# klindsay28/Newton-Krylov_OOC

Measured on AMD Instinct MI355X. Metric: GMRES JVPs/sec, py_driver_2d iage (value = value_frozen: products on frozen years, the default; value_reference_semantic: the reference's product, two free-running years, same solver, same run), higher is better.
Workload: dtype f64

## Files before the change

### newton-krylov_ooc_amd/csrc/nk2d_api.hip

```cpp
#include "nk2d_common.h"
#include "nk2d_build_id.h"

#include <algorithm>
#include <cmath>
#include <cstring>
#include <new>

namespace {

template <typename T>
int dev_alloc(nk2d_ctx* c, T** p, size_t n) {
    NK2D_CHECK(c, hipMalloc((void**)p, sizeof(T) * std::max<size_t>(n, 1)));
    NK2D_CHECK(c, hipMemsetAsync(*p, 0, sizeof(T) * std::max<size_t>(n, 1), nk2d_s(c)));
    return 0;
}

int ensure_stage(nk2d_ctx* c, size_t n) {
    if (n <= c->stage_elems) return 0;
    NK2D_CHECK(c, hipStreamSynchronize(nk2d_s(c)));
    if (c->STAGE) NK2D_CHECK(c, hipFree(c->STAGE));
    if (c->hSTAGE) NK2D_CHECK(c, hipHostFree(c->hSTAGE));
    c->STAGE = c->hSTAGE = nullptr;
    c->stage_elems = 0;
    NK2D_CHECK(c, hipMalloc((void**)&c->STAGE, sizeof(double) * n));
// ... 191 lines not shown
    }
    if (key == "pc_panel") {
        if (value != 32.0 && value != 64.0) return nk2d_fail(c, "nk2d_set_option: pc_panel is 32 or 64");
        c->pc_panel = (int)value;
        return 0;
    }
    if (key == "final_fuse") { c->final_fuse = value != 0.0; return 0; }
    if (key == "year_fences") { c->year_fences = value != 0.0; return 0; }
    if (key == "frozen_persistent") { c->frozen_persistent = value != 0.0; return 0; }
    if (key == "frozen_team") { c->frozen_team = value != 0.0; return 0; }
    if (key == "frozen_coef_lds") { c->frozen_coef_lds = (int)value & 63; return 0; }
    if (key == "frozen_sums_poison") { c->frozen_sums_poison = (int)value != 0 ? 1 : 0; return 0; }
    if (key == "frozen_early") { c->frozen_early = (int)value != 0 ? 1 : 0; return 0; }
    if (key == "frozen_stage_exchange") { c->frozen_stage_exchange = (int)value != 0 ? 1 : 0; return 0; }
    if (key == "frozen_xlane") { c->frozen_xlane = (int)value != 0 ? 1 : 0; return 0; }
    if (key == "frozen_by_column") { c->frozen_by_column = (int)value; return 0; }
    if (key == "frozen_cache_after") { c->frozen_cache_after = (int)value; return 0; }
    if (key == "spec_bias") { c->spec_bias = value > 0.0 ? value : 1.0; return 0; }
    if (key == "stream_years") { c->stream_years = (int)value; c->stream_lost = 0; return 0; }
    if (key == "frozen_tape") {
        if (value != 0.0 && value != 1.0) return nk2d_fail(c, "nk2d_set_option: frozen_tape is 0 or 1");
        c->frozen_tape = (int)value;
        return 0;
    }
    if (key == "stream_hist") {
        if (value != 0.0 && value != 1.0) return nk2d_fail(c, "nk2d_set_option: stream_hist is 0 or 1");
        c->stream_hist = (int)value;
        return 0;
    }
    if (key == "stream_hist_mb") {
// ... 406 lines not shown
    c->frozen_forced_years = 0;
    c->frozen_phosphorus = 0;
    c->frozen_phosphorus_shallow = 0;
    c->frozen_phosphorus_shallow_years = 0;
    c->frozen_two_waves_last = 0;
    c->frozen_phosphorus_years = c->frozen_two_waves_years = 0;
    c->frozen_cache_piece_allocs = c->frozen_cache_early_requests = 0;
    c->frozen_coef_lds = 63;
    c->frozen_lds_bits = 0;
    c->frozen_early = NK2D_FROZEN_EARLY_DEFAULT;
    c->frozen_early_bits = 0;
    c->frozen_stage_exchange = NK2D_FROZEN_STAGE_EXCHANGE_DEFAULT;
    c->frozen_stage_exchange_bits = 0;
    c->frozen_xlane = NK2D_FROZEN_XLANE_DEFAULT;
    c->frozen_xlane_bits = 0;
    c->stream_xlane = 0;
    c->stream_xlane_bits = 0;
    c->frozen_by_column = 1;
    c->strm = nullptr;
    c->spec_bias = 1.0;
    c->stream_two_waves = std::getenv("NK2D_STREAM_TWO_WAVES") ? std::atoi(std::getenv("NK2D_STREAM_TWO_WAVES")) : 1;
    c->stream_years = 1;
    c->stream_on = 0;
    c->stream_lost = 0;
    c->stream_cmds = c->stream_launches = c->stream_timeouts = c->stream_years_run = 0;
    c->frozen_tape = 0;
    c->tape = nullptr;
    c->tape_rec = c->tape_foreign = 0;
    c->tape_years_run = c->tape_builds = c->tape_timeouts = c->tape_fallbacks = 0;
    c->frozen_wpb = 2;
// ... 498 lines not shown
        int w = -1, row = -1, lane = -1;
        if (std::sscanf(key.c_str() + 15, "%d_%d_%d", &w, &row, &lane) != 3 || w < 0 || w > 1 || row < 0 || row >= NK2D_XLANE_SELFTEST_ROWS ||
            lane < 0 || lane > 63)
            return nk2d_fail(c, "nk2d_get_counter: unknown counter " + key);
        v = xl_selftest_out[((size_t)w * NK2D_XLANE_SELFTEST_ROWS + row) * 64 + lane];
    }
    else if (key == "frozen_launch_us") v = c->frozen_launch_us;
    else if (key == "frozen_cache_pending") v = nk2d_frozen_cache_pending(c);
    else if (key == "frozen_cache_bytes") v = nk2d_frozen_cache_bytes(c);
    else if (key == "frozen_cache_pieces") v = nk2d_frozen_cache_npieces(c);
    else if (key == "frozen_cache_lean") v = nk2d_frozen_cache_is_lean(c);
    else if (key == "frozen_lds_bits") v = c->frozen_lds_bits;
    else if (key == "frozen_early_bits") v = c->frozen_early_bits;
    else if (key == "frozen_stage_exchange_bits") v = c->frozen_stage_exchange_bits;
    else if (key == "frozen_xlane_bits") v = c->frozen_xlane_bits;
    else if (key == "stream_xlane_bits") v = c->stream_xlane_bits;
    else if (key == "frozen_step_sums_hash") v = c->frozen_step_sums_hash;
    else if (key == "frozen_lean_years") v = c->frozen_lean_years;
    else if (key == "frozen_forced_years") v = c->frozen_forced_years;
    else if (key == "frozen_phosphorus_years") v = c->frozen_phosphorus_years;
    else if (key == "frozen_phosphorus_shallow_years") v = c->frozen_phosphorus_shallow_years;
    else if (key == "frozen_two_waves_years") v = c->frozen_two_waves_years;
    else if (key == "frozen_cache_piece_allocs") v = nk2d_frozen_cache_piece_allocs(c);
    else if (key == "frozen_cache_early_requests") v = c->frozen_cache_early_requests;
    else if (key == "frozen_fallbacks") v = c->frozen_fallbacks;
    else if (key == "frozen_resumes") v = c->frozen_resumes;
    else if (key == "spec_launches_dropped") v = c->cnt_spec_dropped;
    else if (key == "spec_front_launches_dropped") v = c->cnt_front_dropped;
    else if (key == "err_estimates_queued") v = c->cnt_err_queued;
    else if (key == "err_estimates_dropped") v = c->cnt_err_void;
// ... 331 lines not shown
```

### newton-krylov_ooc_amd/csrc/nk2d_bodies.h

```cpp
#pragma once
#include <atomic>
#include <chrono>
#include <cmath>
#include <cstdio>
#include <cstdlib>
#include <cstring>
#include <mutex>
#include <thread>

#include "nk2d_common.h"
#include "nk2d_hostmath.h"


struct DevP {
    int nz, ny, tc, ncol;
    const double *VV, *KH, *WT, *WB, *DZR, *ZM0, *ZM1, *DM, *DMR, *DYR, *BLDMAX;
    double surf[NK2D_MAX_TRACERS], starget[NK2D_MAX_TRACERS], decay[NK2D_MAX_TRACERS], csrc;
    double atol, rtol;
    double ph_hs, ph_mu, ph_sig, ph_rd, ph_rp, ph_vs;
    const double *LIGHT, *UPR;
    const double *SMSREC, *RESTREC;
    int f_sms, f_restore;
    double f_thres_r;
    size_t np;
// ... 1912 lines not shown
                }
                __builtin_amdgcn_s_sleep(1);
            }
            if (lane == 0) *lds_ok = good;
#ifdef NK2D_FROZEN_CLOCKS
            ck_wait += (long long)__builtin_amdgcn_s_memrealtime() - ck_flag;
#endif
        }
        __syncthreads();
#ifdef NK2D_FROZEN_CLOCKS
        ck_match = (long long)__builtin_amdgcn_s_memrealtime();
#endif
        if (fences) __builtin_amdgcn_fence(__ATOMIC_ACQUIRE, "agent");
        return *lds_ok != 0;
    }
    __device__ __forceinline__ bool sync() {
        asm volatile("s_waitcnt vmcnt(0)" ::: "memory");
        if (fences) __builtin_amdgcn_fence(__ATOMIC_RELEASE, "agent");
        __syncthreads();
        ++phase;
        if (threadIdx.x < 64) {
            const int lane = threadIdx.x;
            if (lane == 0) __hip_atomic_store(flags + (size_t)me * 32, phase, __ATOMIC_RELAXED, __HIP_MEMORY_SCOPE_AGENT);
            const int other = (lane == 0) ? left : ((lane == 1) ? right : -1);
            int good = 1;
            long long spins = 0;
            const long long t_begin = (long long)__builtin_amdgcn_s_memrealtime();
            for (;;) {
                unsigned v = phase;
                if (other >= 0) v = __hip_atomic_load(flags + (size_t)other * 32, __ATOMIC_RELAXED, __HIP_MEMORY_SCOPE_AGENT);
// ... 239 lines not shown
    int fences;
    int coef_lds;
#define NK2D_FROZEN_EARLY_OF(coef_lds) (((coef_lds) >> 8) & 1)
#define NK2D_FROZEN_XCHG_OF(coef_lds) (((coef_lds) >> 9) & 1)
#define NK2D_FROZEN_XLANE_OF(coef_lds) (((coef_lds) >> 10) & 1)
    int by_column;
    const double* SRC;
    int upr_on;
};

struct FrozenPieceArgs : FrozenArgs {
    PieceTab T;
};
template <int PIECES> struct FrozenArgOf { typedef FrozenArgs type; };
template <> struct FrozenArgOf<1> { typedef FrozenPieceArgs type; };

template <int E, int KIND, int MP>
__device__ __forceinline__ void tend_at_body(const DevP& P, const double* __restrict__ y, const double* __restrict__ kvp,
                                             double* __restrict__ f, int task, int lane) {
    const int tr = task / P.ny, j = task - tr * P.ny;
    const int cs_col = (j > 0) ? task - 1 : task, cn_col = (j < P.ny - 1) ? task + 1 : task;
    ColCoef<E> cf;
    load_coef<E>(P, j, lane, cf);
    double c[E], cs[E], cn[E], kv[E], ff[E];
    load_col<E, MP>(y, task, lane, c);
    load_col<E, MP>(y, cs_col, lane, cs);
    load_col<E, MP>(y, cn_col, lane, cn);
    load_col<E, MP>(kvp, j, lane, kv);
    tend_col<E, KIND>(P, cf, c, cs, cn, kv, tr, lane, ff);
    if constexpr (KIND == 2) forced_sources<E>(P, kvp, j, lane, c, ff);
// ... 56 lines not shown
```

### newton-krylov_ooc_amd/csrc/nk2d_common.h

```cpp
#pragma once

#include <hip/hip_runtime.h>
#include <stdint.h>
#include <string>
#include <mutex>
#include <vector>

#include "../../include/nk2d.h"

#define NK2D_WAVE 64
#define NK2D_WAVES_PER_BLOCK 4
#define NK2D_BLOCK (NK2D_WAVE * NK2D_WAVES_PER_BLOCK)
#define NK2D_MAX_E 8
#define NK2D_OWN_REC_CAP 65536
#define NK2D_CKPT_EVERY 128


#define NK2D_FROZEN_EARLY_DEFAULT 1
#define NK2D_FROZEN_STAGE_EXCHANGE_DEFAULT 1
#define NK2D_FROZEN_XLANE_DEFAULT 1
#ifndef NK2D_FROZEN_XLANE_MOVES
#define NK2D_FROZEN_XLANE_MOVES 97
#endif
struct nk2d_ctx {
    nk2d_desc d;
    int nz, ny, tc, E, nzp, ncol, nreg;
    int kind;
    size_t nv;
    size_t np;
    int dev;
    hipStream_t stream_;
    std::string err;
    struct nk2d_stream_state* strm;
    int stream_years;
    int stream_two_waves;
// ... 61 lines not shown
    void* frozen_cache;
    int frozen_persistent;
    int frozen_persistent_max_e;
    double frozen_cache_max_gb;
    int64_t frozen_cache_builds, frozen_persistent_years;
    int frozen_team;
    int frozen_wpb;
    int frozen_coef_lds;
    int frozen_lds_bits;
    int frozen_early;
    int frozen_early_bits;
    int frozen_stage_exchange;
    int frozen_stage_exchange_bits;
    int frozen_xlane;
    int frozen_xlane_bits;
    int frozen_by_column;
    int frozen_alloc_async;
    int frozen_cache_after;
    int frozen_cache_pieces;
    double frozen_cache_piece_mb;
    int64_t frozen_cache_piece_rows;
    int frozen_cache_lean;
    int64_t frozen_lean_years;
    uint64_t frozen_lean_mem_key;
    int frozen_forced;
    int64_t frozen_forced_years;
    int frozen_phosphorus;
    int frozen_phosphorus_shallow;
    int64_t frozen_phosphorus_shallow_years;
    int frozen_two_waves_last;
// ... 621 lines not shown
```

### newton-krylov_ooc_amd/csrc/nk2d_frozen.hip

```cpp
#include "nk2d_bodies.h"
#include "nk2d_frozen_plan.h"

#include <algorithm>
#ifdef NK2D_FROZEN_CLOCKS
#include <cstdio>
#endif
#include <vector>

__device__ __forceinline__ RowTabs cache_row_tabs(const CachePiecePtrs& C, int i) {
    const int p = i / C.T.rows;
    return piece_row_tabs(C.C, C.T, C.T.base[p], i - p * C.T.rows);
}

template <int E, int PIECES = 0>
__global__ void __launch_bounds__(NK2D_BLOCK) k_cache_planes(DevP P, const CacheRow* __restrict__ rows, typename CacheArgOf<PIECES>::type C, int n) {
    const int lane = threadIdx.x & 63;
    const long long task = (long long)blockIdx.x * (blockDim.x >> 6) + (threadIdx.x >> 6);
    const long long per_row = 4LL * P.ny;
    if (task >= per_row * n) return;
    const int i = (int)(task / per_row), rem = (int)(task - (long long)i * per_row);
    const int slot = rem / P.ny, j = rem - slot * P.ny;
    const CacheRow& R = rows[i];
    if (slot < 3) {
        double kv[E];
// ... 56 lines not shown
__device__ __forceinline__ void frozen_factor_phase(const DevP& P, const FusedArgs& FA, int wave, int lane, const FinalArgs* fin, const LdsSrc* L,
                                                    int coef_lds, bool w_in_lds, double* piv_lds) {
    if (w_in_lds) newton_fused_body<E, KIND, 1, 1, MPX, FINAL, 3>(P, FA, wave, lane, fin, L);
    else if (coef_lds) newton_fused_body<E, KIND, 1, 1, MPX, FINAL, 1>(P, FA, wave, lane, fin, L);
    else newton_fused_body<E, KIND, 1, 1, MPX, FINAL>(P, FA, wave, lane, fin);
    if (piv_lds) {
        asm volatile("s_waitcnt vmcnt(0)" ::: "memory");
        double v[E];
        load_col<E>(FA.sw.fr_inv, wave, lane, v);
        w_lds_put<E>(piv_lds, 0, lane, v);
    }
}

template <int E, int KIND, int TEAM = 0, int PIECES = 0, int LEAN = 0>
__global__ void __launch_bounds__(NK2D_BLOCK) k_frozen_persistent(DevP P, typename FrozenArgOf<PIECES>::type A) {
#include "nk2d_frozen_body.inc"
}
template <int E, int PIECES>
__global__ void __launch_bounds__(NK2D_BLOCK) __attribute__((amdgpu_waves_per_eu(2, 2))) k_frozen_persistent_w2(DevP P, typename FrozenArgOf<PIECES>::type A) {
    constexpr int KIND = 1, TEAM = 0, LEAN = 1;
#include "nk2d_frozen_body.inc"
}

struct nk2d_frozen_cache {
    uint64_t key = 0;
    int64_t n = 0;
    std::vector<double*> blocks;
    size_t block_rows = 0;
    bool pieces = false, lean = false, src = false;
    double** blocks_dev = nullptr;
    size_t blocks_dev_cap = 0;
    CacheRow* rows_dev = nullptr;
    FrozenRow* frows_dev = nullptr;
    size_t rows_cap = 0;
    std::vector<FrozenRow> frows;
    double* lean_tab = nullptr;
// ... 143 lines not shown
static hipError_t launch_resident(nk2d_ctx* c, K kernel, dim3 grid, dim3 block, DevP& P, ARGS& A, size_t lds_bytes = 0, bool check_only = false) {
    int per_cu = 0;
    hipError_t rc = hipOccupancyMaxActiveBlocksPerMultiprocessor(&per_cu, kernel, (int)block.x, lds_bytes);
    if (rc != hipSuccess) return rc;
    hipDeviceProp_t prop;
    rc = hipGetDeviceProperties(&prop, c->dev);
    if (rc != hipSuccess) return rc;
    if ((long long)per_cu * prop.multiProcessorCount < (long long)grid.x) return hipErrorCooperativeLaunchTooLarge;
    if (check_only) return hipSuccess;
    if (std::getenv("NK2D_DIAG_COOPERATIVE")) {
        void* args[2] = {&P, &A};
        return hipLaunchCooperativeKernel((const void*)kernel, grid, block, args, (unsigned)lds_bytes, nk2d_s(c));
    }
    hipLaunchKernelGGL(kernel, grid, block, lds_bytes, nk2d_s(c), P, A);
    return hipGetLastError();
}

template <int E, int KIND, int TEAM, int PIECES, int LEAN>
static hipError_t launch_frozen_one(nk2d_ctx* c, dim3 grid, DevP& P, typename FrozenArgOf<PIECES>::type& A) {
    const int wpb = TEAM ? NK2D_WAVES_PER_BLOCK : std::max(1, std::min(NK2D_WAVES_PER_BLOCK, c->frozen_wpb));
    const dim3 g = TEAM ? grid : dim3((unsigned)((c->ncol + wpb - 1) / wpb));
    if (!TEAM && E >= 3 && A.by_column)
        return launch_resident(c, k_frozen_persistent<E, KIND, TEAM, PIECES, LEAN>, dim3((unsigned)c->ny), dim3(64 * c->tc), P, A,
                               sizeof(double) * frozen_lds_doubles(E, A.coef_lds, true, c->tc));
    const size_t lds = (!TEAM && E >= 3 && A.coef_lds) ? sizeof(double) * frozen_lds_doubles(E, A.coef_lds, false, wpb) : 0;
    return launch_resident(c, k_frozen_persistent<E, KIND, TEAM, PIECES, LEAN>, g, dim3(64 * wpb), P, A, lds);
}
template <int KIND, int TEAM, int PIECES, int LEAN>
static hipError_t launch_frozen_e(nk2d_ctx* c, dim3 grid, DevP& P, typename FrozenArgOf<PIECES>::type& A) {
    switch (c->E) {
// ... 321 lines not shown
    A.upr_on = (pl.src || pl.phos) ? 1 : 0;
    A.SRC = (pl.src && !pl.pieces) ? fc->blocks[0] + L.oS : nullptr;
    *P = make_devp(c);
    if (pl.src || pl.phos) P->UPR = fc->upr;
    NK2D_TRY(frozen_fit_lds(c, in, pl, &A.coef_lds, &A.by_column));
    c->frozen_lds_bits = A.coef_lds;
    c->frozen_early_bits = (A.coef_lds & 48) == 48 ? c->frozen_early : 0;
    A.coef_lds |= c->frozen_early_bits << 8;
    const bool team_year = c->frozen_team && c->E <= 2 && !pl.phos;
    c->frozen_stage_exchange_bits =
        ((A.coef_lds & 48) == 48 && NK2D_FROZEN_XCHG(c->E, c->kind, team_year, pl.pieces, pl.lean)) ? c->frozen_stage_exchange : 0;
    A.coef_lds |= c->frozen_stage_exchange_bits << 9;
    c->frozen_xlane_bits =
        (c->frozen_stage_exchange_bits != 0 && NK2D_FROZEN_XLANE(c->E, c->kind, team_year, pl.pieces, pl.lean)) ? c->frozen_xlane : 0;
    A.coef_lds |= c->frozen_xlane_bits << 10;
    return 0;
}

static int frozen_launch_year(nk2d_ctx* c, const FrozenPlan& pl, int64_t n, DevP& P, FrozenPieceArgs& A) {
    const bool team = c->frozen_team && c->E <= 2 && !pl.phos;
    const dim3 grid((unsigned)(team ? c->ncol : nk2d_grid(c->ncol)));
    NK2D_CHECK(c, hipMemsetAsync(c->YR_SYNC, 0, yr_sync_bytes(c), nk2d_s(c)));
    NK2D_CHECK(c, hipMemsetAsync(c->YR_OUT, 0, sizeof(double) * 32, nk2d_s(c)));
    NK2D_CHECK(c, hipEventRecord(c->yr_ev[0], nk2d_s(c)));
    {
        struct Turn {
            int waves;
            explicit Turn(int w) : waves(w) { nk2d_turn_take(waves); }
            ~Turn() { nk2d_turn_give(waves); }
        } turn(team ? 4 * c->ncol : c->ncol);
        hipError_t rc = hipErrorInvalidValue;
        bool two = false;
        if (pl.phos) rc = launch_frozen_phos_flavour(c, pl.pieces, P, A, false, &two);
        else if (pl.lean) rc = pl.pieces ? launch_frozen<1, 1>(c, team, grid, P, A) : launch_frozen<0, 1>(c, team, grid, P, static_cast<FrozenArgs&>(A));
        else rc = pl.pieces ? launch_frozen<1, 0>(c, team, grid, P, A) : launch_frozen<0, 0>(c, team, grid, P, static_cast<FrozenArgs&>(A));
        c->frozen_two_waves_last = two ? 1 : 0;
        if (rc == hipErrorCooperativeLaunchTooLarge) { (void)hipGetLastError(); return 1; }
        NK2D_CHECK(c, rc);
        NK2D_CHECK(c, hipEventRecord(c->yr_ev[1], nk2d_s(c)));
        NK2D_CHECK(c, hipMemcpyAsync(c->hYR_OUT, c->YR_OUT, sizeof(double) * 32, hipMemcpyDeviceToHost, nk2d_s(c)));
        NK2D_CHECK(c, hipStreamSynchronize(nk2d_s(c)));
    }
    const double* o = c->hYR_OUT;
    if ((int)o[0] != 0 || (int64_t)o[1] != n) return 2;
#ifdef NK2D_FROZEN_CLOCKS
    std::fprintf(stderr, "frozen clocks (early %d, stage exchange %d, xlane %d): %.0f phases, per phase drain %.3f us, flag store to poll match %.3f us, "
                 "poll match to neighbours loaded %.3f us, rest %.3f us; kernel %.3f ms\n",
                 c->frozen_early_bits, c->frozen_stage_exchange_bits, c->frozen_xlane_bits, o[11], 0.01 * o[8] / o[11], 0.01 * o[9] / o[11], 0.01 * o[12] / o[11],
// ... 75 lines not shown
```

### newton-krylov_ooc_amd/csrc/nk2d_frozen_body.inc

```
    constexpr int XCD = 0, NB = 1;
    __shared__ int lds_ok;
    __shared__ double team_lds[TEAM ? sizeof(TeamLds<E, 3>) / sizeof(double) : 1];
    constexpr int MPX = XCD ? 2 : 1;
    const int lane = threadIdx.x & 63;
    int wg = (int)blockIdx.x;
    const int tw = uni_i((int)(threadIdx.x >> 6));
    const bool by_col = !TEAM && !XCD && NB != 0 && A.by_column != 0;
    const int wave = TEAM ? uni_i(wg) : (by_col ? uni_i(tw * P.ny + wg) : uni_i(wg * (int)(blockDim.x >> 6) + (int)(threadIdx.x >> 6)));
    const bool col_wave = wave < P.ncol && (!by_col || (tw < P.tc && wg < P.ny));
    int nb_left, nb_right;
    if constexpr (TEAM) {
        const int nb_j = wave % P.ny;
        nb_left = (nb_j > 0) ? wg - 1 : -1;
        nb_right = (nb_j < P.ny - 1) ? wg + 1 : -1;
    } else if (by_col) {
        nb_left = (wg > 0) ? wg - 1 : -1;
        nb_right = (wg < P.ny - 1) ? wg + 1 : -1;
    } else {
        const int wpb = (int)(blockDim.x >> 6);
        const int c0 = wg * wpb, cl = min(c0 + wpb - 1, P.ncol - 1);
        nb_left = (c0 % P.ny > 0) ? wg - 1 : -1;
        nb_right = (cl % P.ny < P.ny - 1) ? wg + 1 : -1;
    }
    NeighbourSync nbs{(unsigned*)((char*)A.arrive + 8192), A.abort_flag, wg, nb_left, nb_right, 0u, &lds_ok, A.spin_ticks, A.fences};
// ... 6 lines not shown
    (void)pc_p; (void)pc_r;
#define FZ_Y (swapY ? A.YOLD : A.Y)
#define FZ_YOLD (swapY ? A.Y : A.YOLD)
#define FZ_Z (swapZ ? A.ZN : A.Z)
#define FZ_ZN (swapZ ? A.Z : A.ZN)
#define FZ_SYNC() \
    if (!nbs.sync()) { status = 1; goto finish; }
#define FZ_OWN_DEAD() \
    if constexpr (OWN) { \
        _Pragma("unroll") for (int r_ = 0; r_ < 3; ++r_) { \
            _Pragma("unroll") for (int e_ = 0; e_ < E; ++e_) own.z[r_][e_] = 0.0; \
        } \
    }
    constexpr bool COEF_LDS = NB != 0 && !TEAM && !XCD && E >= 3;
    extern __shared__ double dyn_lds[];
    const bool w_in_lds = COEF_LDS && (A.coef_lds & 2) != 0;
    const bool step_in_lds = COEF_LDS && by_col && (A.coef_lds & 4) != 0;
    const bool piv_in_lds = COEF_LDS && by_col && (A.coef_lds & 8) != 0;
    constexpr bool OWN = COEF_LDS && NK2D_FROZEN_OWN(E, KIND, TEAM, LEAN);
    const int own_bits = OWN && by_col ? (A.coef_lds & 48) : 0;
    (void)own_bits;
    const int nwv = (int)(blockDim.x >> 6);
    double* my_coef;
    double* my_w;
    double* step_lds = nullptr;
    double* my_piv = nullptr;
    double* my_y = nullptr;
    if (by_col) {
        double* p = dyn_lds;
        my_coef = p; p += NK2D_COEF_LDS_DOUBLES(E);
        step_lds = p; p += step_in_lds ? 5 * E * 64 : 0;
        my_w = p + (size_t)tw * (3 * E * 64); p += w_in_lds ? (size_t)nwv * 3 * E * 64 : 0;
        my_piv = p + (size_t)tw * (E * 64); p += piv_in_lds ? (size_t)nwv * E * 64 : 0;
        my_y = p + (size_t)tw * (E * 64);
    } else {
// ... 9 lines not shown
        for (int r = 0; r < 3; ++r) {
#pragma unroll
            for (int e = 0; e < E; ++e) own.z[r][e] = 0.0;
        }
    }
    if constexpr (COEF_LDS) {
        if (A.coef_lds && col_wave && (!by_col || tw == 0)) {
            ColCoef<E> cf;
            load_coef<E>(P, wave % P.ny, lane, cf);
            store_coef_lds<E>(my_coef, lane, cf);
        }
        if (by_col && A.coef_lds) __syncthreads();
    }
    int lds_step = -1;
    (void)lds_step;
    LateNorm late = {0.0, nullptr, (OWN && by_col && own_bits == 48) ? uni_i(NK2D_FROZEN_EARLY_OF(A.coef_lds)) : 0, 0};
    (void)late;
    constexpr bool XCHG = OWN && NK2D_FROZEN_XCHG(E, KIND, TEAM, PIECES, LEAN);
    const int xchg = (XCHG && by_col && own_bits == 48) ? uni_i(NK2D_FROZEN_XCHG_OF(A.coef_lds)) : 0;
    double* const xu0 = XCHG ? (double*)((char*)A.arrive + yr_xchg_offset(P.ncol)) : nullptr;
    (void)xchg; (void)xu0;
    constexpr bool XLANE = XCHG && NK2D_FROZEN_XLANE(E, KIND, TEAM, PIECES, LEAN);
    const int xlane = (XLANE && xchg) ? uni_i(NK2D_FROZEN_XLANE_OF(A.coef_lds)) : 0;
    (void)xlane;
#define FZ_U (swapZ ? xu0 + 3 * nv : xu0)
#define FZ_UN (swapZ ? xu0 : xu0 + 3 * nv)
    if (col_wave && (!TEAM || tw == 0)) {
        double zero[E];
#pragma unroll
        for (int e = 0; e < E; ++e) zero[e] = 0.0;
        if constexpr (XCHG) {
            if (xchg) {
                double y0[E];
                load_col<E, MPX>(FZ_Y, wave, lane, y0);
#pragma unroll
                for (int e = 0; e < E; ++e) y0[e] = y0[e] + zero[e];
#pragma unroll
                for (int i = 0; i < 3; ++i) store_col<E, 1>(FZ_U + i * nv, wave, lane, y0);
            }
// ... 102 lines not shown
                        }
                        }
                        lds_step = i;
                        __syncthreads();
                    }
                }
#ifdef NK2D_FROZEN_CLOCKS
                late.ck_match = nbs.ck_match;
#endif
                if (is_final) {
                    FinalArgs Fin;
                    Fin.ynew = FZ_YOLD;
                    Fin.znext = do_stage ? FZ_ZN : FZ_Z;
                    Fin.x0 = R.x0; Fin.x1 = R.x1; Fin.x2 = R.x2;
                    Fin.nblk_cols = 0;
                    if constexpr (TEAM) {
                        if constexpr (LEAN) {
                            if (col_wave && fac)
                                newton_team_body<E, KIND, 1, 1, 4, 1, MPX>(PK, FA, *reinterpret_cast<TeamLds<E, 3>*>(team_lds), wave, tw, lane, &Fin);
                        }
                        if (col_wave && !fac)
                            newton_team_body<E, KIND, 0, 1, 4, 1, MPX>(P, FA, *reinterpret_cast<TeamLds<E, 3>*>(team_lds), wave, tw, lane, &Fin);
                    } else if (col_wave && fac) {
                        if constexpr (LEAN && COEF_LDS) frozen_factor_phase<E, KIND, MPX, 1>(PK, FA, wave, lane, &Fin, &L, A.coef_lds, w_in_lds, piv_in_lds ? my_piv : nullptr);
                        else if constexpr (LEAN) newton_fused_body<E, KIND, 1, 1, MPX, 1>(PK, FA, wave, lane, &Fin);
                    } else if (col_wave) {
                        bool taken = false;
                        if constexpr (KIND == 0 && E <= 2) {
                            if (m == 1) { newton_single_body<E, MPX, 1>(P, FA, wave, lane, &Fin); taken = true; }
                        }
// ... 9 lines not shown
                            }
                            if (taken) {}
                            else if (own_bits == 48) { newton_fused_body<E, KIND, 0, 1, MPX, 1, 191>(P, FA, wave, lane, &Fin, &L, &own, &late); taken = true; }
                            else if (!PIECES && own_bits == 32) { newton_fused_body<E, KIND, 0, 1, MPX, 1, 47>(P, FA, wave, lane, &Fin, &L, &own); taken = true; }
                            else if (own_bits == 16) { newton_fused_body<E, KIND, 0, 1, MPX, 1, 31>(P, FA, wave, lane, &Fin, &L, &own); FZ_OWN_DEAD() taken = true; }
                        }
                        if constexpr (COEF_LDS) {
                            if (taken) {}
                            else if (step_in_lds && piv_in_lds) { newton_fused_body<E, KIND, 0, 1, MPX, 1, 15>(P, FA, wave, lane, &Fin, &L); FZ_OWN_DEAD() taken = true; }
                            else if (step_in_lds) { newton_fused_body<E, KIND, 0, 1, MPX, 1, 7>(P, FA, wave, lane, &Fin, &L); FZ_OWN_DEAD() taken = true; }
                            else if (w_in_lds) { newton_fused_body<E, KIND, 0, 1, MPX, 1, 3>(P, FA, wave, lane, &Fin, &L); FZ_OWN_DEAD() taken = true; }
                            else if (A.coef_lds) { newton_fused_body<E, KIND, 0, 1, MPX, 1, 1>(P, FA, wave, lane, &Fin, &L); FZ_OWN_DEAD() taken = true; }
                        }
                        if (!taken) { newton_fused_body<E, KIND, 0, 1, MPX, 1>(P, FA, wave, lane, &Fin); FZ_OWN_DEAD() }
                    }
                    swapY ^= 1;
                    if (do_stage) swapZ ^= 1;
                } else {
                    if constexpr (TEAM) {
                        if constexpr (LEAN) {
                            if (col_wave && fac)
                                newton_team_body<E, KIND, 1, 1, 4, 0, MPX>(PK, FA, *reinterpret_cast<TeamLds<E, 3>*>(team_lds), wave, tw, lane, nullptr);
                        }
                        if (col_wave && !fac)
                            newton_team_body<E, KIND, 0, 1, 4, 0, MPX>(P, FA, *reinterpret_cast<TeamLds<E, 3>*>(team_lds), wave, tw, lane, nullptr);
                    } else if (col_wave && fac) {
                        if constexpr (LEAN && COEF_LDS) frozen_factor_phase<E, KIND, MPX, 0>(PK, FA, wave, lane, nullptr, &L, A.coef_lds, w_in_lds, piv_in_lds ? my_piv : nullptr);
                        else if constexpr (LEAN) newton_fused_body<E, KIND, 1, 1, MPX, 0>(PK, FA, wave, lane);
                    } else if (col_wave) {
                        bool taken = false;
                        if constexpr (KIND == 0 && E <= 2) {
                            if (m == 1) { newton_single_body<E, MPX, 0>(P, FA, wave, lane); taken = true; }
                        }
// ... 9 lines not shown
                            }
                            if (taken) {}
                            else if (own_bits == 48) { newton_fused_body<E, KIND, 0, 1, MPX, 0, 191>(P, FA, wave, lane, nullptr, &L, &own, &late); taken = true; }
                            else if (!PIECES && own_bits == 32) { newton_fused_body<E, KIND, 0, 1, MPX, 0, 47>(P, FA, wave, lane, nullptr, &L, &own); taken = true; }
                            else if (own_bits == 16) { newton_fused_body<E, KIND, 0, 1, MPX, 0, 31>(P, FA, wave, lane, nullptr, &L, &own); FZ_OWN_DEAD() taken = true; }
                        }
                        if constexpr (COEF_LDS) {
                            if (taken) {}
                            else if (step_in_lds && piv_in_lds) { newton_fused_body<E, KIND, 0, 1, MPX, 0, 15>(P, FA, wave, lane, nullptr, &L); FZ_OWN_DEAD() taken = true; }
                            else if (step_in_lds) { newton_fused_body<E, KIND, 0, 1, MPX, 0, 7>(P, FA, wave, lane, nullptr, &L); FZ_OWN_DEAD() taken = true; }
                            else if (w_in_lds) { newton_fused_body<E, KIND, 0, 1, MPX, 0, 3>(P, FA, wave, lane, nullptr, &L); FZ_OWN_DEAD() taken = true; }
                            else if (A.coef_lds) { newton_fused_body<E, KIND, 0, 1, MPX, 0, 1>(P, FA, wave, lane, nullptr, &L); FZ_OWN_DEAD() taken = true; }
                        }
                        if (!taken) { newton_fused_body<E, KIND, 0, 1, MPX, 0>(P, FA, wave, lane); FZ_OWN_DEAD() }
                    }
                    if (do_stage && do_update) swapZ ^= 1;
                }
                src = 1 - src;
                if constexpr (OWN) {
                    nbs.publish();
                    if (late.pending) {
                        if (lane == 0) st_mp<MPX>(late.part, late.acc);
                        late.pending = 0;
                    }
                    if (!nbs.wait()) { status = 1; goto finish; }
                } else {
                    FZ_SYNC()
                }
            }
        }
        if (with_err) {
            if (col_wave && (!TEAM || tw == 0)) {
                ErrArgs EA = {};
                EA.sw.JL = J; EA.sw.JU = J + A.C.np; EA.sw.JS = J + 2 * A.C.np; EA.sw.JN = J + 3 * A.C.np; EA.sw.JC = J + 4 * A.C.np;
                EA.sw.fr_inv = LEAN ? A.C.fr_inv : (PIECES ? T.fr_inv : A.C.fr_inv + (size_t)i * nv);
                EA.sw.fr_tab = LEAN ? A.C.fr_tab : (PIECES ? T.fr_tab : A.C.fr_tab + (size_t)i * A.C.ntab);
                EA.sw.xr_old = A.XR[0]; EA.sw.xr_new = A.XR[1];
                EA.f = A.F; EA.z = FZ_Z; EA.y = FZ_Y; EA.nv = nv; EA.h = R.h;
                EA.part = A.STEP_PART + (size_t)(3 * i + 2) * P.ncol;
                EA.stage = 0; EA.last = 1;
// ... 64 lines not shown
```

### newton-krylov_ooc_amd/csrc/nk2d_frozen_plan.h

```cpp
#pragma once

#include <algorithm>
#include <cmath>
#include <cstddef>
#include <cstdint>
#include <initializer_list>

#define NK2D_WAVES_PER_BLOCK 4
#define NK2D_TAB 14
#define NK2D_SCHED_WIDTH 8
#define NK2D_COEF_LDS_DOUBLES(E) ((7 * (E) + 1) * 64)

#define NK2D_FROZEN_OWN(E, KIND, TEAM, LEAN) ((E) >= 5 && (E) <= 7 && ((KIND) == 0 || (KIND) == 2) && !(TEAM) && !(LEAN))
#define NK2D_FROZEN_XCHG(E, KIND, TEAM, PIECES, LEAN) (NK2D_FROZEN_OWN(E, KIND, TEAM, LEAN) && !((E) == 7 && (KIND) == 0 && (PIECES)))
#define NK2D_FROZEN_XLANE(E, KIND, TEAM, PIECES, LEAN) (NK2D_FROZEN_XCHG(E, KIND, TEAM, PIECES, LEAN) && !((E) == 6 && (KIND) == 0 && (PIECES)))

struct FrozenPlanIn {
    int E, kind, tc, ny, ncol;
    size_t np, nv, kv_len;
    int sms_nrec;
    double sink_thres, t0;
    int frozen_persistent, frozen_persistent_max_e, frozen_forced, frozen_phosphorus;
    int frozen_phosphorus_shallow;
    int frozen_cache_lean, frozen_cache_pieces;
    double frozen_cache_piece_mb;
    int64_t frozen_cache_piece_rows;
    double frozen_cache_max_gb;
    int frozen_cache_after, frozen_alloc_async, frozen_err_check;
    int frozen_coef_lds, frozen_by_column, frozen_wpb, frozen_team;
    int factor_fp32, jac_stage_state, hist_n;
// ... 232 lines not shown
```

### newton-krylov_ooc_amd/csrc/nk2d_radau.hip

```cpp
#include "nk2d_common.h"
#include "nk2d_stream.h"

#include <algorithm>
#include <chrono>
#include <cmath>
#include <cstring>
#include <limits>
#include <string>
#include <vector>

namespace {

const double RC[3] = {0.15505102572168222, 0.6449489742783178, 1.0};
const double MU_REAL = 3.637834252744496;
const double MU_CR = 2.6810828736277523, MU_CI = -3.050430199247411;
const int NEWTON_MAXITER = 6;
const double MIN_FACTOR = 0.2, MAX_FACTOR = 10.0;

struct Ctl {
    nk2d_ctx* c;
    double t, t1;
    double h_abs, h_abs_old, err_old;
    bool has_old_h, has_old_err;
    bool current_jac, have_lu, have_dense;
// ... 981 lines not shown
    };
    if (!s.no_persistent && !c->stream_on) {
        std::vector<char> sampled;
        const int prc = nk2d_frozen_persistent(c, sched, n, &sampled);
        if (prc < 0) return prc;
        if (prc == 0) {
            const double* r = sched + (n - 1) * NK2D_SCHED_WIDTH;
            s.t = r[0];
            NK2D_TRY(commit_step(s, r[0], r[1]));
            NK2D_TRY(fetch_sums(0));
            if (first_unconverged(sched, 0) < 0) {
                const int64_t bad_err = first_bad_err(sched, 0, -1, sampled);
                if (bad_err >= 0) return err_failure(bad_err);
                c->frozen_persistent_years++;
                if (nk2d_frozen_cache_is_lean(c)) c->frozen_lean_years++;
                if (c->kind == 2 && (c->E > 4 || (c->d.sms_nrec > 0 && c->d.sink_thres > 0.0))) c->frozen_forced_years++;
                if (c->kind == 1) { c->frozen_phosphorus_years++; c->frozen_two_waves_years += c->frozen_two_waves_last; }
                if (c->kind == 1 && c->E <= 2) c->frozen_phosphorus_shallow_years++;
                return 0;
            }
            return 3;
        }
        if (prc == 2) {
            c->st.nbarrier_timeouts++;
            if (c->kind == 1) c->frozen_fallbacks++;
            return 3;
        }
    }
    int64_t start = 0;
    std::vector<char> err_done((size_t)n, 0);
// ... 215 lines not shown
```

### newton-krylov_ooc_amd/engine.py

```python

import ctypes
import os

import numpy as np

from . import _lib
from .grid import BLDEPTH_MIN, YEAR, bldepth_time_knots


DEFAULT_LIN_TOL = 3.0e-2
DEFAULT_JAC_FRESH = 1
DEFAULT_JAC_STAGE = 1
DEFAULT_GROWTH_CAP = 0.0


def phos_pc_fused_from_env():
    return int(os.environ.get("NK2D_PHOS_PC_FUSED", "0")) != 0


class Nk2dError(RuntimeError):
    pass


class Nk2dFrozenMismatch(Nk2dError):
# ... 163 lines not shown
            self.set_option("frozen_cache_early", float(os.environ["NK2D_FROZEN_CACHE_EARLY"]))
        if "NK2D_FROZEN_CACHE_LEAN" in os.environ:
            self.set_option("frozen_cache_lean", float(os.environ["NK2D_FROZEN_CACHE_LEAN"]))
        if "NK2D_FROZEN_FORCED" in os.environ:
            self.set_option("frozen_forced", float(os.environ["NK2D_FROZEN_FORCED"]))
        if "NK2D_FROZEN_PHOSPHORUS" in os.environ:
            self.set_option("frozen_phosphorus", float(os.environ["NK2D_FROZEN_PHOSPHORUS"]))
        if "NK2D_FROZEN_PHOSPHORUS_SHALLOW" in os.environ:
            self.set_option("frozen_phosphorus_shallow", float(os.environ["NK2D_FROZEN_PHOSPHORUS_SHALLOW"]))
        if "NK2D_FROZEN_EARLY" in os.environ:
            self.set_option("frozen_early", float(os.environ["NK2D_FROZEN_EARLY"]))
        if "NK2D_FROZEN_STAGE_EXCHANGE" in os.environ:
            self.set_option("frozen_stage_exchange", float(os.environ["NK2D_FROZEN_STAGE_EXCHANGE"]))
        if "NK2D_FROZEN_XLANE" in os.environ:
            self.set_option("frozen_xlane", float(os.environ["NK2D_FROZEN_XLANE"]))
        if "NK2D_STREAM_XLANE" in os.environ:
            self.set_option("stream_xlane", float(os.environ["NK2D_STREAM_XLANE"]))
        if "NK2D_PC_TWO_ENDED" in os.environ:
            self.set_option("pc_two_ended", float(os.environ["NK2D_PC_TWO_ENDED"]))
        if "NK2D_PC_PIVOT_WAVE" in os.environ:
            self.set_option("pc_pivot_wave", float(os.environ["NK2D_PC_PIVOT_WAVE"]))
        if "NK2D_PC_PANEL" in os.environ:
            self.set_option("pc_panel", float(os.environ["NK2D_PC_PANEL"]))
        self.set_option("jac_fresh", float(os.environ.get("NK2D_JAC_FRESH", DEFAULT_JAC_FRESH)))
        self.set_option("growth_cap", float(os.environ.get("NK2D_GROWTH_CAP", DEFAULT_GROWTH_CAP)))
        self.set_option("jac_stage", float(os.environ.get("NK2D_JAC_STAGE", DEFAULT_JAC_STAGE)))

    @property
    def _ctx(self):
        if self._handle is None:
# ... 494 lines not shown
```

Baseline: 8.991.

## Add dedicated specialized frozen persistent kernel with single-load neighbor polling

Adds a separate persistent kernel entry compiled only for the default frozen-year configuration, with the runtime LDS, early-norm, stage-exchange and cross-lane choices fixed as constants. This strips dead branches, which should cut register pressure and instruction overhead. Mode 2, the default, also swaps the neighbor barrier wait for a variant where lanes 0-2 each issue one atomic load per spin, reading both neighbors' flags and the abort flag together. The risk is that residency is checked through occupancy, and a launch that fails or does not fit leaves the year without a launched kernel rather than using the generic path.

```diff
diff --git a/newton-krylov_ooc_amd/csrc/nk2d_api.hip b/newton-krylov_ooc_amd/csrc/nk2d_api.hip
--- a/newton-krylov_ooc_amd/csrc/nk2d_api.hip
+++ b/newton-krylov_ooc_amd/csrc/nk2d_api.hip
@@ -229,6 +229,11 @@
     if (key == "frozen_early") { c->frozen_early = (int)value != 0 ? 1 : 0; return 0; }
     if (key == "frozen_stage_exchange") { c->frozen_stage_exchange = (int)value != 0 ? 1 : 0; return 0; }
     if (key == "frozen_xlane") { c->frozen_xlane = (int)value != 0 ? 1 : 0; return 0; }
+    if (key == "frozen_dedicated") {
+        if (value != 0.0 && value != 1.0 && value != 2.0) return nk2d_fail(c, "nk2d_set_option: frozen_dedicated is 0, 1 or 2");
+        c->frozen_dedicated = (int)value;
+        return 0;
+    }
     if (key == "frozen_by_column") { c->frozen_by_column = (int)value; return 0; }
     if (key == "frozen_cache_after") { c->frozen_cache_after = (int)value; return 0; }
     if (key == "spec_bias") { c->spec_bias = value > 0.0 ? value : 1.0; return 0; }
@@ -665,6 +670,9 @@
     c->frozen_stage_exchange_bits = 0;
     c->frozen_xlane = NK2D_FROZEN_XLANE_DEFAULT;
     c->frozen_xlane_bits = 0;
+    c->frozen_dedicated = NK2D_FROZEN_DEDICATED_DEFAULT;
+    c->frozen_dedicated_bits = 0;
+    c->frozen_dedicated_years = 0;
     c->stream_xlane = 0;
     c->stream_xlane_bits = 0;
     c->frozen_by_column = 1;
@@ -1193,6 +1201,8 @@
     else if (key == "frozen_early_bits") v = c->frozen_early_bits;
     else if (key == "frozen_stage_exchange_bits") v = c->frozen_stage_exchange_bits;
     else if (key == "frozen_xlane_bits") v = c->frozen_xlane_bits;
+    else if (key == "frozen_dedicated_bits") v = c->frozen_dedicated_bits;
+    else if (key == "frozen_dedicated_years") v = c->frozen_dedicated_years;
     else if (key == "stream_xlane_bits") v = c->stream_xlane_bits;
     else if (key == "frozen_step_sums_hash") v = c->frozen_step_sums_hash;
     else if (key == "frozen_lean_years") v = c->frozen_lean_years;
diff --git a/newton-krylov_ooc_amd/csrc/nk2d_bodies.h b/newton-krylov_ooc_amd/csrc/nk2d_bodies.h
--- a/newton-krylov_ooc_amd/csrc/nk2d_bodies.h
+++ b/newton-krylov_ooc_amd/csrc/nk2d_bodies.h
@@ -1950,6 +1950,41 @@
         if (fences) __builtin_amdgcn_fence(__ATOMIC_ACQUIRE, "agent");
         return *lds_ok != 0;
     }
+    __device__ __forceinline__ bool wait_one_load() {
+        if (threadIdx.x < 64) {
+            const int lane = threadIdx.x;
+            const int other = (lane == 0) ? left : ((lane == 1) ? right : -1);
+            const unsigned* const src = (lane == 2) ? (const unsigned*)abort_flag : ((other >= 0) ? flags + (size_t)other * 32 : nullptr);
+            int good = 1;
+            long long spins = 0;
+            const long long t_begin = (long long)__builtin_amdgcn_s_memrealtime();
+            for (;;) {
+                unsigned got = 0;
+                if (src != nullptr) got = __hip_atomic_load(src, __ATOMIC_RELAXED, __HIP_MEMORY_SCOPE_AGENT);
+                const unsigned v = (other >= 0) ? got : phase;
+                if (__all((int)(v >= phase))) break;
+                const int ab = __builtin_amdgcn_readlane((int)got, 2);
+                const bool late = ((++spins & 63) == 0 || spin_ticks == 0) &&
+                                  (long long)__builtin_amdgcn_s_memrealtime() - t_begin > spin_ticks;
+                if (late || spins > 4000LL * NK2D_SPIN_LIMIT || ab != 0) {
+                    if (lane == 0) __hip_atomic_store(abort_flag, 1, __ATOMIC_RELAXED, __HIP_MEMORY_SCOPE_AGENT);
+                    good = 0;
+                    break;
+                }
+                __builtin_amdgcn_s_sleep(1);
+            }
+            if (lane == 0) *lds_ok = good;
+#ifdef NK2D_FROZEN_CLOCKS
+            ck_wait += (long long)__builtin_amdgcn_s_memrealtime() - ck_flag;
+#endif
+        }
+        __syncthreads();
+#ifdef NK2D_FROZEN_CLOCKS
+        ck_match = (long long)__builtin_amdgcn_s_memrealtime();
+#endif
+        if (fences) __builtin_amdgcn_fence(__ATOMIC_ACQUIRE, "agent");
+        return *lds_ok != 0;
+    }
     __device__ __forceinline__ bool sync() {
         asm volatile("s_waitcnt vmcnt(0)" ::: "memory");
         if (fences) __builtin_amdgcn_fence(__ATOMIC_RELEASE, "agent");
@@ -2219,6 +2254,7 @@
 };
 template <int PIECES> struct FrozenArgOf { typedef FrozenArgs type; };
 template <> struct FrozenArgOf<1> { typedef FrozenPieceArgs type; };
+hipError_t nk2d_frozen_launch_d(nk2d_ctx* c, dim3 grid, dim3 block, DevP& P, FrozenPieceArgs& A, bool pieces, int* max_blocks, size_t lds_bytes);
 
 template <int E, int KIND, int MP>
 __device__ __forceinline__ void tend_at_body(const DevP& P, const double* __restrict__ y, const double* __restrict__ kvp,
diff --git a/newton-krylov_ooc_amd/csrc/nk2d_common.h b/newton-krylov_ooc_amd/csrc/nk2d_common.h
--- a/newton-krylov_ooc_amd/csrc/nk2d_common.h
+++ b/newton-krylov_ooc_amd/csrc/nk2d_common.h
@@ -19,6 +19,7 @@
 #define NK2D_FROZEN_EARLY_DEFAULT 1
 #define NK2D_FROZEN_STAGE_EXCHANGE_DEFAULT 1
 #define NK2D_FROZEN_XLANE_DEFAULT 1
+#define NK2D_FROZEN_DEDICATED_DEFAULT 2
 #ifndef NK2D_FROZEN_XLANE_MOVES
 #define NK2D_FROZEN_XLANE_MOVES 97
 #endif
@@ -110,6 +111,9 @@
     int frozen_stage_exchange_bits;
     int frozen_xlane;
     int frozen_xlane_bits;
+    int frozen_dedicated;
+    int frozen_dedicated_bits;
+    int64_t frozen_dedicated_years;
     int frozen_by_column;
     int frozen_alloc_async;
     int frozen_cache_after;
diff --git a/newton-krylov_ooc_amd/csrc/nk2d_frozen.hip b/newton-krylov_ooc_amd/csrc/nk2d_frozen.hip
--- a/newton-krylov_ooc_amd/csrc/nk2d_frozen.hip
+++ b/newton-krylov_ooc_amd/csrc/nk2d_frozen.hip
@@ -94,12 +94,16 @@
 
 template <int E, int KIND, int TEAM = 0, int PIECES = 0, int LEAN = 0>
 __global__ void __launch_bounds__(NK2D_BLOCK) k_frozen_persistent(DevP P, typename FrozenArgOf<PIECES>::type A) {
+#define FZ_ONLY 0
 #include "nk2d_frozen_body.inc"
+#undef FZ_ONLY
 }
 template <int E, int PIECES>
 __global__ void __launch_bounds__(NK2D_BLOCK) __attribute__((amdgpu_waves_per_eu(2, 2))) k_frozen_persistent_w2(DevP P, typename FrozenArgOf<PIECES>::type A) {
     constexpr int KIND = 1, TEAM = 0, LEAN = 1;
+#define FZ_ONLY 0
 #include "nk2d_frozen_body.inc"
+#undef FZ_ONLY
 }
 
 struct nk2d_frozen_cache {
@@ -273,6 +277,20 @@
     }
     hipLaunchKernelGGL(kernel, grid, block, lds_bytes, nk2d_s(c), P, A);
     return hipGetLastError();
+}
+
+static hipError_t launch_resident_dedicated(nk2d_ctx* c, bool pieces, DevP& P, FrozenPieceArgs& A) {
+    if (!A.by_column || c->tc > NK2D_WAVES_PER_BLOCK) return hipErrorInvalidValue;
+    const dim3 grid((unsigned)c->ny), block((unsigned)(64 * c->tc));
+    const size_t lds_bytes = sizeof(double) * frozen_lds_doubles(c->E, A.coef_lds, true, c->tc);
+    int per_cu = 0;
+    hipError_t rc = nk2d_frozen_launch_d(c, grid, block, P, A, pieces, &per_cu, lds_bytes);
+    if (rc != hipSuccess) return rc;
+    hipDeviceProp_t prop;
+    rc = hipGetDeviceProperties(&prop, c->dev);
+    if (rc != hipSuccess) return rc;
+    if ((long long)per_cu * prop.multiProcessorCount < (long long)grid.x) return hipErrorCooperativeLaunchTooLarge;
+    return nk2d_frozen_launch_d(c, grid, block, P, A, pieces, nullptr, lds_bytes);
 }
 
 template <int E, int KIND, int TEAM, int PIECES, int LEAN>
@@ -624,6 +642,9 @@
     c->frozen_xlane_bits =
         (c->frozen_stage_exchange_bits != 0 && NK2D_FROZEN_XLANE(c->E, c->kind, team_year, pl.pieces, pl.lean)) ? c->frozen_xlane : 0;
     A.coef_lds |= c->frozen_xlane_bits << 10;
+    c->frozen_dedicated_bits = frozen_dedicated(c->frozen_dedicated, c->E, c->kind, team_year, pl.pieces, pl.lean, c->frozen_lds_bits,
+                                                c->frozen_early_bits, c->frozen_stage_exchange_bits, c->frozen_xlane_bits);
+    if (c->frozen_dedicated_bits == 2) A.coef_lds |= 1 << 11;
     return 0;
 }
 
@@ -641,7 +662,8 @@
         } turn(team ? 4 * c->ncol : c->ncol);
         hipError_t rc = hipErrorInvalidValue;
         bool two = false;
-        if (pl.phos) rc = launch_frozen_phos_flavour(c, pl.pieces, P, A, false, &two);
+        if (c->frozen_dedicated_bits != 0) rc = launch_resident_dedicated(c, pl.pieces, P, A);
+        else if (pl.phos) rc = launch_frozen_phos_flavour(c, pl.pieces, P, A, false, &two);
         else if (pl.lean) rc = pl.pieces ? launch_frozen<1, 1>(c, team, grid, P, A) : launch_frozen<0, 1>(c, team, grid, P, static_cast<FrozenArgs&>(A));
         else rc = pl.pieces ? launch_frozen<1, 0>(c, team, grid, P, A) : launch_frozen<0, 0>(c, team, grid, P, static_cast<FrozenArgs&>(A));
         c->frozen_two_waves_last = two ? 1 : 0;
diff --git a/newton-krylov_ooc_amd/csrc/nk2d_frozen_body.inc b/newton-krylov_ooc_amd/csrc/nk2d_frozen_body.inc
--- a/newton-krylov_ooc_amd/csrc/nk2d_frozen_body.inc
+++ b/newton-krylov_ooc_amd/csrc/nk2d_frozen_body.inc
@@ -1,3 +1,6 @@
+#if FZ_ONLY
+    static_assert(FZ_ONLY == 959 && !TEAM && !LEAN && NK2D_FROZEN_OWN(E, KIND, TEAM, LEAN), "the dedicated entry: the one body of the default year");
+#endif
     constexpr int XCD = 0, NB = 1;
     __shared__ int lds_ok;
     __shared__ double team_lds[TEAM ? sizeof(TeamLds<E, 3>) / sizeof(double) : 1];
@@ -5,7 +8,12 @@
     const int lane = threadIdx.x & 63;
     int wg = (int)blockIdx.x;
     const int tw = uni_i((int)(threadIdx.x >> 6));
+#if FZ_ONLY
+    (void)team_lds;
+    constexpr bool by_col = true;
+#else
     const bool by_col = !TEAM && !XCD && NB != 0 && A.by_column != 0;
+#endif
     const int wave = TEAM ? uni_i(wg) : (by_col ? uni_i(tw * P.ny + wg) : uni_i(wg * (int)(blockDim.x >> 6) + (int)(threadIdx.x >> 6)));
     const bool col_wave = wave < P.ncol && (!by_col || (tw < P.tc && wg < P.ny));
     int nb_left, nb_right;
@@ -44,11 +52,19 @@
     }
     constexpr bool COEF_LDS = NB != 0 && !TEAM && !XCD && E >= 3;
     extern __shared__ double dyn_lds[];
+#if FZ_ONLY
+    constexpr bool w_in_lds = true, step_in_lds = true, piv_in_lds = true;
+#else
     const bool w_in_lds = COEF_LDS && (A.coef_lds & 2) != 0;
     const bool step_in_lds = COEF_LDS && by_col && (A.coef_lds & 4) != 0;
     const bool piv_in_lds = COEF_LDS && by_col && (A.coef_lds & 8) != 0;
+#endif
     constexpr bool OWN = COEF_LDS && NK2D_FROZEN_OWN(E, KIND, TEAM, LEAN);
+#if FZ_ONLY
+    constexpr int own_bits = 48;
+#else
     const int own_bits = OWN && by_col ? (A.coef_lds & 48) : 0;
+#endif
     (void)own_bits;
     const int nwv = (int)(blockDim.x >> 6);
     double* my_coef;
@@ -88,15 +104,28 @@
     }
     int lds_step = -1;
     (void)lds_step;
+#if FZ_ONLY
+    LateNorm late = {0.0, nullptr, 1, 0};
+#else
     LateNorm late = {0.0, nullptr, (OWN && by_col && own_bits == 48) ? uni_i(NK2D_FROZEN_EARLY_OF(A.coef_lds)) : 0, 0};
+#endif
     (void)late;
+#if FZ_ONLY
+    constexpr bool XCHG = OWN;
+    constexpr int xchg = 1;
+#else
     constexpr bool XCHG = OWN && NK2D_FROZEN_XCHG(E, KIND, TEAM, PIECES, LEAN);
     const int xchg = (XCHG && by_col && own_bits == 48) ? uni_i(NK2D_FROZEN_XCHG_OF(A.coef_lds)) : 0;
+#endif
     double* const xu0 = XCHG ? (double*)((char*)A.arrive + yr_xchg_offset(P.ncol)) : nullptr;
     (void)xchg; (void)xu0;
+#if FZ_ONLY
+    const int poll_one = uni_i((A.coef_lds >> 11) & 1);
+#else
     constexpr bool XLANE = XCHG && NK2D_FROZEN_XLANE(E, KIND, TEAM, PIECES, LEAN);
     const int xlane = (XLANE && xchg) ? uni_i(NK2D_FROZEN_XLANE_OF(A.coef_lds)) : 0;
     (void)xlane;
+#endif
 #define FZ_U (swapZ ? xu0 + 3 * nv : xu0)
 #define FZ_UN (swapZ ? xu0 : xu0 + 3 * nv)
     if (col_wave && (!TEAM || tw == 0)) {
@@ -229,6 +258,13 @@
                     Fin.znext = do_stage ? FZ_ZN : FZ_Z;
                     Fin.x0 = R.x0; Fin.x1 = R.x1; Fin.x2 = R.x2;
                     Fin.nblk_cols = 0;
+#if FZ_ONLY
+                    (void)fac;
+                    if (col_wave) {
+                        const StageXchg XC = {FZ_U, do_stage ? FZ_UN : FZ_U, 0};
+                        newton_fused_body<E, KIND, 0, 1, MPX, 1, FZ_ONLY>(P, FA, wave, lane, &Fin, &L, &own, &late, &XC);
+                    }
+#else
                     if constexpr (TEAM) {
                         if constexpr (LEAN) {
                             if (col_wave && fac)
@@ -268,9 +304,17 @@
                         }
                         if (!taken) { newton_fused_body<E, KIND, 0, 1, MPX, 1>(P, FA, wave, lane, &Fin); FZ_OWN_DEAD() }
                     }
+#endif
                     swapY ^= 1;
                     if (do_stage) swapZ ^= 1;
                 } else {
+#if FZ_ONLY
+                    (void)fac;
+                    if (col_wave) {
+                        const StageXchg XC = {FZ_U, (do_stage && do_update) ? FZ_UN : FZ_U, (with_err || last_row) ? 1 : 0};
+                        newton_fused_body<E, KIND, 0, 1, MPX, 0, FZ_ONLY>(P, FA, wave, lane, nullptr, &L, &own, &late, &XC);
+                    }
+#else
                     if constexpr (TEAM) {
                         if constexpr (LEAN) {
                             if (col_wave && fac)
@@ -310,6 +354,7 @@
                         }
                         if (!taken) { newton_fused_body<E, KIND, 0, 1, MPX, 0>(P, FA, wave, lane); FZ_OWN_DEAD() }
                     }
+#endif
                     if (do_stage && do_update) swapZ ^= 1;
                 }
                 src = 1 - src;
@@ -319,7 +364,11 @@
                         if (lane == 0) st_mp<MPX>(late.part, late.acc);
                         late.pending = 0;
                     }
+#if FZ_ONLY
+                    if (!(poll_one ? nbs.wait_one_load() : nbs.wait())) { status = 1; goto finish; }
+#else
                     if (!nbs.wait()) { status = 1; goto finish; }
+#endif
                 } else {
                     FZ_SYNC()
                 }
diff --git a/newton-krylov_ooc_amd/csrc/nk2d_frozen_d.hip b/newton-krylov_ooc_amd/csrc/nk2d_frozen_d.hip
--- /dev/null
+++ b/newton-krylov_ooc_amd/csrc/nk2d_frozen_d.hip
@@ -0,0 +1,43 @@
+#include "nk2d_bodies.h"
+#include "nk2d_frozen_plan.h"
+
+template <int E, int KIND, int PIECES>
+__global__ void __launch_bounds__(NK2D_BLOCK) k_frozen_persistent_d(DevP P, typename FrozenArgOf<PIECES>::type A) {
+    constexpr int TEAM = 0, LEAN = 0;
+#define FZ_ONLY 959
+#include "nk2d_frozen_body.inc"
+#undef FZ_ONLY
+}
+
+template <int E, int KIND, int PIECES>
+static hipError_t frozen_launch_d_one(nk2d_ctx* c, dim3 grid, dim3 block, DevP& P, typename FrozenArgOf<PIECES>::type& A, int* max_blocks,
+                                      size_t lds_bytes) {
+    if constexpr (NK2D_FROZEN_DEDICATED(E, KIND, PIECES)) {
+        if (max_blocks) return hipOccupancyMaxActiveBlocksPerMultiprocessor(max_blocks, k_frozen_persistent_d<E, KIND, PIECES>, (int)block.x, lds_bytes);
+        hipLaunchKernelGGL((k_frozen_persistent_d<E, KIND, PIECES>), grid, block, lds_bytes, nk2d_s(c), P, A);
+        return hipGetLastError();
+    } else {
+        return hipErrorInvalidValue;
+    }
+}
+
+template <int E, int KIND>
+static hipError_t frozen_launch_d_ek(nk2d_ctx* c, dim3 grid, dim3 block, DevP& P, FrozenPieceArgs& A, bool pieces, int* max_blocks, size_t lds_bytes) {
+    if (pieces) return frozen_launch_d_one<E, KIND, 1>(c, grid, block, P, A, max_blocks, lds_bytes);
+    return frozen_launch_d_one<E, KIND, 0>(c, grid, block, P, static_cast<FrozenArgs&>(A), max_blocks, lds_bytes);
+}
+
+hipError_t nk2d_frozen_launch_d(nk2d_ctx* c, dim3 grid, dim3 block, DevP& P, FrozenPieceArgs& A, bool pieces, int* max_blocks, size_t lds_bytes) {
+    const bool forced = c->kind == 2;
+    if (c->kind != 0 && !forced) return hipErrorInvalidValue;
+    switch (c->E) {
+        case 5: return forced ? frozen_launch_d_ek<5, 2>(c, grid, block, P, A, pieces, max_blocks, lds_bytes)
+                              : frozen_launch_d_ek<5, 0>(c, grid, block, P, A, pieces, max_blocks, lds_bytes);
+        case 6: return forced ? frozen_launch_d_ek<6, 2>(c, grid, block, P, A, pieces, max_blocks, lds_bytes)
+                              : frozen_launch_d_ek<6, 0>(c, grid, block, P, A, pieces, max_blocks, lds_bytes);
+        case 7: return forced ? frozen_launch_d_ek<7, 2>(c, grid, block, P, A, pieces, max_blocks, lds_bytes)
+                              : frozen_launch_d_ek<7, 0>(c, grid, block, P, A, pieces, max_blocks, lds_bytes);
+        default: break;
+    }
+    return hipErrorInvalidValue;
+}
diff --git a/newton-krylov_ooc_amd/csrc/nk2d_frozen_plan.h b/newton-krylov_ooc_amd/csrc/nk2d_frozen_plan.h
--- a/newton-krylov_ooc_amd/csrc/nk2d_frozen_plan.h
+++ b/newton-krylov_ooc_amd/csrc/nk2d_frozen_plan.h
@@ -14,6 +14,15 @@
 #define NK2D_FROZEN_OWN(E, KIND, TEAM, LEAN) ((E) >= 5 && (E) <= 7 && ((KIND) == 0 || (KIND) == 2) && !(TEAM) && !(LEAN))
 #define NK2D_FROZEN_XCHG(E, KIND, TEAM, PIECES, LEAN) (NK2D_FROZEN_OWN(E, KIND, TEAM, LEAN) && !((E) == 7 && (KIND) == 0 && (PIECES)))
 #define NK2D_FROZEN_XLANE(E, KIND, TEAM, PIECES, LEAN) (NK2D_FROZEN_XCHG(E, KIND, TEAM, PIECES, LEAN) && !((E) == 6 && (KIND) == 0 && (PIECES)))
+#define NK2D_FROZEN_DEDICATED(E, KIND, PIECES) NK2D_FROZEN_XLANE(E, KIND, 0, PIECES, 0)
+
+static inline int frozen_dedicated(int option, int E, int kind, bool team, bool pieces, bool lean, int lds_bits, int early_bits,
+                                   int stage_exchange_bits, int xlane_bits) {
+    if (option != 1 && option != 2) return 0;
+    if (team || lean || !NK2D_FROZEN_DEDICATED(E, kind, pieces ? 1 : 0)) return 0;
+    if (lds_bits != 63 || early_bits != 1 || stage_exchange_bits != 1 || xlane_bits != 1) return 0;
+    return option;
+}
 
 struct FrozenPlanIn {
     int E, kind, tc, ny, ncol;
diff --git a/newton-krylov_ooc_amd/csrc/nk2d_radau.hip b/newton-krylov_ooc_amd/csrc/nk2d_radau.hip
--- a/newton-krylov_ooc_amd/csrc/nk2d_radau.hip
+++ b/newton-krylov_ooc_amd/csrc/nk2d_radau.hip
@@ -1019,6 +1019,7 @@
                 if (bad_err >= 0) return err_failure(bad_err);
                 c->frozen_persistent_years++;
                 if (nk2d_frozen_cache_is_lean(c)) c->frozen_lean_years++;
+                if (c->frozen_dedicated_bits != 0) c->frozen_dedicated_years++;
                 if (c->kind == 2 && (c->E > 4 || (c->d.sms_nrec > 0 && c->d.sink_thres > 0.0))) c->frozen_forced_years++;
                 if (c->kind == 1) { c->frozen_phosphorus_years++; c->frozen_two_waves_years += c->frozen_two_waves_last; }
                 if (c->kind == 1 && c->E <= 2) c->frozen_phosphorus_shallow_years++;
diff --git a/newton-krylov_ooc_amd/engine.py b/newton-krylov_ooc_amd/engine.py
--- a/newton-krylov_ooc_amd/engine.py
+++ b/newton-krylov_ooc_amd/engine.py
@@ -201,6 +201,8 @@
             self.set_option("frozen_stage_exchange", float(os.environ["NK2D_FROZEN_STAGE_EXCHANGE"]))
         if "NK2D_FROZEN_XLANE" in os.environ:
             self.set_option("frozen_xlane", float(os.environ["NK2D_FROZEN_XLANE"]))
+        if "NK2D_FROZEN_DEDICATED" in os.environ:
+            self.set_option("frozen_dedicated", float(os.environ["NK2D_FROZEN_DEDICATED"]))
         if "NK2D_STREAM_XLANE" in os.environ:
             self.set_option("stream_xlane", float(os.environ["NK2D_STREAM_XLANE"]))
         if "NK2D_PC_TWO_ENDED" in os.environ:
```

Result: faster. 9.185 (median of 6 runs) (+2.2%).
